# CloudEngineHub/FairyGen

Hardware: AMD Instinct MI355X
Metric: decoded frames/sec (sec/clip in config), Wan2.2-TI2V-5B 704x1280x121 @ 5 steps (higher is better)
Workload: dtype bf16

## Files before the change

fairygen_amd/csrc/capi.cpp:

```cpp
#include <stdarg.h>
#include <stdio.h>
#include "../../include/fairygen_hip.h"

static thread_local char g_err[512] = "";

void fg_set_error(const char* fmt, ...) {
    va_list ap;
    va_start(ap, fmt);
    vsnprintf(g_err, sizeof(g_err), fmt, ap);
    va_end(ap);
}

extern "C" int fg_version(void) { return 5; }
extern "C" const char* fg_last_error(void) { return g_err; }
```

fairygen_amd/csrc/dit_elementwise.hip:

```cpp
#include "common.h"

#ifndef FG_ROW_MIN_WAVES
#define FG_ROW_MIN_WAVES 4
#endif
#define FG_ROW_BOUNDS __launch_bounds__(256, FG_ROW_MIN_WAVES)

namespace {

constexpr int kMaxVec = 8;
constexpr int kRowsPerBlock = 4;

struct Row {
    float v[kMaxVec][8];
};

__device__ __forceinline__ void load_row(const bf16* p, int C, int lane, Row& r) {
    const int nvec = C >> 3;
#pragma unroll
    for (int i = 0; i < kMaxVec; ++i) {
        const int vi = lane + i * 64;
        if (vi < nvec) {
            bf16x8 t = *reinterpret_cast<const bf16x8*>(p + (int64_t)vi * 8);
#pragma unroll
            for (int j = 0; j < 8; ++j) r.v[i][j] = (float)t[j];
        } else {
#pragma unroll
            for (int j = 0; j < 8; ++j) r.v[i][j] = 0.f;
        }
    }
}

__device__ __forceinline__ bf16x8 ld8(const bf16* p) { return *reinterpret_cast<const bf16x8*>(p); }
__device__ __forceinline__ void st8(bf16* p, const float* f) {
    bf16x8 t;
#pragma unroll
    for (int j = 0; j < 8; ++j) t[j] = (bf16)f[j];
    *reinterpret_cast<bf16x8*>(p) = t;
}
// ... 238 lines not shown
                const int d0 = PLAIN ? ((vi * 8) & (head_dim - 1)) : ((vi * 8) % head_dim);
                if (F32TAB) {
                    f32x4 t0 = h0, t1 = h1;
                    if (!hoist) {
                        const f32x4* tp = reinterpret_cast<const f32x4*>(static_cast<const float*>(ctv) + (row * half + (d0 >> 1)) * 2);
                        t0 = tp[0];
                        t1 = tp[1];
                    }
                    const float cs[8] = {t0[0], t0[1], t0[2], t0[3], t1[0], t1[1], t1[2], t1[3]};
#pragma unroll
                    for (int j = 0; j < 4; ++j) {
                        const float a = o[2 * j], b = o[2 * j + 1], c = cs[2 * j], sn = cs[2 * j + 1];
                        o[2 * j] = rbf(__builtin_fmaf(a, c, -(b * sn)));
                        o[2 * j + 1] = rbf(__builtin_fmaf(a, sn, b * c));
                    }
                } else {
                    const double* cp = static_cast<const double*>(ctv) + row * half + (d0 >> 1);
                    const double* sp = static_cast<const double*>(stv) + row * half + (d0 >> 1);
#pragma unroll
                    for (int j = 0; j < 4; ++j) {
                        const double a = (double)o[2 * j], b = (double)o[2 * j + 1];
                        const double c = cp[j], sn = sp[j];
                        o[2 * j] = (float)(bf16)(a * c - b * sn);
                        o[2 * j + 1] = (float)(bf16)(a * sn + b * c);
                    }
                }
            }
            const int col = vi * 8, g = PLAIN ? 0 : col / group_cols;
            st8(out + g * out_group_stride + row * out_ld + (col - g * group_cols), o);
        }
    }
}

__global__ __launch_bounds__(256) void copy_groups_kernel(const bf16* __restrict__ src, int64_t sgs, int64_t sld,
                                                          bf16* __restrict__ dst, int64_t dgs, int64_t dld, int groups,
                                                          int64_t rows, int vec_per_row) {
    const int64_t total = (int64_t)groups * rows * vec_per_row;
    for (int64_t i = (int64_t)blockIdx.x * blockDim.x + threadIdx.x; i < total; i += (int64_t)gridDim.x * blockDim.x) {
        const int64_t rg = i / vec_per_row;
        const int v = (int)(i - rg * vec_per_row);
        const int64_t r = rg / groups;
        const int g = (int)(rg - r * groups);
        *reinterpret_cast<u32x4*>(dst + g * dgs + r * dld + v * 8) =
            *reinterpret_cast<const u32x4*>(src + g * sgs + r * sld + v * 8);
    }
}


template <int KIND>
__global__ __launch_bounds__(256) void act_kernel(const bf16* __restrict__ x, bf16* __restrict__ out, int64_t nvec) {
    for (int64_t i = (int64_t)blockIdx.x * blockDim.x + threadIdx.x; i < nvec; i += (int64_t)gridDim.x * blockDim.x) {
        const bf16x8 v = ld8(x + i * 8);
        float o[8];
#pragma unroll
        for (int j = 0; j < 8; ++j) o[j] = KIND == 0 ? silu_f((float)v[j]) : gelu_tanh_f((float)v[j]);
        st8(out + i * 8, o);
    }
}

__global__ __launch_bounds__(256) void cfg_euler_kernel(const bf16* __restrict__ lat, const bf16* __restrict__ posi,
                                                        const bf16* __restrict__ nega, bf16* __restrict__ out,
                                                        int64_t n, float cfg, float dsigma) {
    for (int64_t i = (int64_t)blockIdx.x * blockDim.x + threadIdx.x; i < n; i += (int64_t)gridDim.x * blockDim.x) {
        const float p = (float)posi[i];
        float pred = p;
        if (nega != nullptr) {
            const float ng = (float)nega[i];
            pred = rbf(ng + rbf(cfg * rbf(p - ng)));
        }
        out[i] = (bf16)((float)lat[i] + rbf(pred * dsigma));
    }
}

inline int check_rows(const char* fn, int64_t rows, int C, int64_t mod_rows, int64_t first_rows) {
    FG_CHECK_ARG(rows >= 0 && C > 0 && (C % 8) == 0 && C <= kMaxVec * 512, "%s: need C %% 8 == 0 and C <= %d (got rows=%lld C=%d)",
                 fn, kMaxVec * 512, (long long)rows, C);
    FG_CHECK_ARG(mod_rows == 1 || mod_rows == 2 || mod_rows == rows, "%s: mod_rows must be 1, 2 or rows (got %lld)", fn,
                 (long long)mod_rows);
    FG_CHECK_ARG(first_rows >= 0 && first_rows <= rows, "%s: first_rows out of range", fn);
    return FG_OK;
}

inline dim3 row_grid(int64_t rows) { return dim3((unsigned)((rows + kRowsPerBlock - 1) / kRowsPerBlock)); }

}

extern "C" {

int fg_ln_modulate_bf16(const void* x, const void* shift, const void* scale, void* out, int64_t rows, int C, float eps,
                        int64_t mod_rows, int64_t first_rows, int64_t mod_ld, fg_stream_t stream) {
    if (int e = check_rows("fg_ln_modulate_bf16", rows, C, mod_rows, first_rows)) return e;
    FG_CHECK_ARG(x && shift && scale && out, "fg_ln_modulate_bf16: null pointer");
    FG_CHECK_ARG(FG_ALIGNED16(x) && FG_ALIGNED16(shift) && FG_ALIGNED16(scale) && FG_ALIGNED16(out) && mod_ld % 8 == 0,
                 "fg_ln_modulate_bf16: pointers / mod_ld must be 16-byte aligned");
    if (rows == 0) return FG_OK;
    hipLaunchKernelGGL(ln_modulate_kernel, row_grid(rows), dim3(256), 0, (hipStream_t)stream, (const bf16*)x,
                       (const bf16*)shift, (const bf16*)scale, (bf16*)out, rows, C, eps, mod_rows, first_rows, mod_ld);
    return fg_launch_status("fg_ln_modulate_bf16");
}

int fg_ln_modulate_fp8_bf16(const void* x, const void* shift, const void* scale, void* out_fp8, float* out_scale, int64_t rows, int C,
                            float eps, int64_t mod_rows, int64_t first_rows, int64_t mod_ld, float fp8_max, fg_stream_t stream) {
    if (int e = check_rows("fg_ln_modulate_fp8_bf16", rows, C, mod_rows, first_rows)) return e;
    FG_CHECK_ARG(x && shift && scale && out_fp8 && out_scale, "fg_ln_modulate_fp8_bf16: null pointer");
    FG_CHECK_ARG(FG_ALIGNED16(x) && FG_ALIGNED16(shift) && FG_ALIGNED16(scale) && (((uintptr_t)out_fp8) & 7) == 0 && mod_ld % 8 == 0 &&
                     fp8_max > 0.f,
                 "fg_ln_modulate_fp8_bf16: pointers / mod_ld must be 16-byte aligned (out_fp8: 8), fp8_max positive");
    if (rows == 0) return FG_OK;
    hipLaunchKernelGGL(ln_modulate_fp8_kernel, row_grid(rows), dim3(256), 0, (hipStream_t)stream, (const bf16*)x, (const bf16*)shift,
                       (const bf16*)scale, (uint8_t*)out_fp8, out_scale, rows, C, eps, mod_rows, first_rows, mod_ld, fp8_max);
    return fg_launch_status("fg_ln_modulate_fp8_bf16");
}

int fg_ln_modulate_dual_bf16(const void* x, const void* shift, const void* scale, void* out, void* out_fp8, float* out_scale,
                             int64_t rows, int C, float eps, int64_t mod_rows, int64_t first_rows, int64_t mod_ld, float fp8_max,
                             fg_stream_t stream) {
    if (int e = check_rows("fg_ln_modulate_dual_bf16", rows, C, mod_rows, first_rows)) return e;
    FG_CHECK_ARG(x && shift && scale && out && out_fp8 && out_scale, "fg_ln_modulate_dual_bf16: null pointer");
    FG_CHECK_ARG(FG_ALIGNED16(x) && FG_ALIGNED16(shift) && FG_ALIGNED16(scale) && FG_ALIGNED16(out) && (((uintptr_t)out_fp8) & 7) == 0 &&
                     mod_ld % 8 == 0 && fp8_max > 0.f,
                 "fg_ln_modulate_dual_bf16: pointers / mod_ld must be 16-byte aligned (out_fp8: 8), fp8_max positive");
    if (rows == 0) return FG_OK;
    hipLaunchKernelGGL(ln_dual_kernel<0>, row_grid(rows), dim3(256), 0, (hipStream_t)stream, (const bf16*)x, (const bf16*)shift,
                       (const bf16*)scale, (bf16*)out, (uint8_t*)out_fp8, out_scale, rows, C, eps, mod_rows, first_rows, mod_ld, fp8_max);
    return fg_launch_status("fg_ln_modulate_dual_bf16");
}

int fg_ln_affine_dual_bf16(const void* x, const void* w, const void* b, void* out, void* out_fp8, float* out_scale, int64_t rows, int C,
// ... 9 lines not shown
    return fg_launch_status("fg_ln_affine_dual_bf16");
}

int fg_residual_ln_fp8_bf16(const void* x, const void* y, const void* gate, void* x_out, const void* p0, const void* p1,
                            void* norm_fp8, float* norm_scale, int mode, int64_t rows, int C, float eps, int64_t mod_rows,
                            int64_t first_rows, int64_t mod_ld, float fp8_max, fg_stream_t stream) {
    FG_CHECK_ARG(mode == 0 || mode == 1, "fg_residual_ln_fp8_bf16: mode must be 0 (modulate) or 1 (affine)");
    const bool need_mod = gate != nullptr || mode == 0;
    if (int e = check_rows("fg_residual_ln_fp8_bf16", rows, C, need_mod ? mod_rows : 1, need_mod ? first_rows : 0)) return e;
    FG_CHECK_ARG(x && y && x_out && p0 && p1 && norm_fp8 && norm_scale, "fg_residual_ln_fp8_bf16: null pointer");
    FG_CHECK_ARG(FG_ALIGNED16(x) && FG_ALIGNED16(y) && FG_ALIGNED16(gate) && FG_ALIGNED16(x_out) && FG_ALIGNED16(p0) &&
                     FG_ALIGNED16(p1) && (((uintptr_t)norm_fp8) & 7) == 0 && mod_ld % 8 == 0 && fp8_max > 0.f,
                 "fg_residual_ln_fp8_bf16: pointers / mod_ld must be 16-byte aligned (norm_fp8: 8), fp8_max positive");
    if (rows == 0) return FG_OK;
    if (!need_mod) { mod_rows = 1; first_rows = 0; }
    if (mode == 0)
        hipLaunchKernelGGL(residual_kernel<0>, row_grid(rows), dim3(256), 0, (hipStream_t)stream, (const bf16*)x,
                           (const bf16*)y, (const bf16*)gate, (bf16*)x_out, (const bf16*)p0, (const bf16*)p1,
                           (bf16*)nullptr, rows, C, eps, mod_rows, first_rows, mod_ld, (uint8_t*)norm_fp8, norm_scale, fp8_max);
    else
        hipLaunchKernelGGL(residual_kernel<1>, row_grid(rows), dim3(256), 0, (hipStream_t)stream, (const bf16*)x,
                           (const bf16*)y, (const bf16*)gate, (bf16*)x_out, (const bf16*)p0, (const bf16*)p1,
                           (bf16*)nullptr, rows, C, eps, mod_rows, first_rows, mod_ld, (uint8_t*)norm_fp8, norm_scale, fp8_max);
    return fg_launch_status("fg_residual_ln_fp8_bf16");
}

int fg_ln_affine_bf16(const void* x, const void* w, const void* b, void* out, int64_t rows, int C, float eps,
                      fg_stream_t stream) {
    if (int e = check_rows("fg_ln_affine_bf16", rows, C, 1, 0)) return e;
    FG_CHECK_ARG(x && w && b && out, "fg_ln_affine_bf16: null pointer");
    FG_CHECK_ARG(FG_ALIGNED16(x) && FG_ALIGNED16(w) && FG_ALIGNED16(b) && FG_ALIGNED16(out),
                 "fg_ln_affine_bf16: pointers must be 16-byte aligned");
    if (rows == 0) return FG_OK;
    hipLaunchKernelGGL(ln_affine_kernel, row_grid(rows), dim3(256), 0, (hipStream_t)stream, (const bf16*)x, (const bf16*)w,
                       (const bf16*)b, (bf16*)out, rows, C, eps);
    return fg_launch_status("fg_ln_affine_bf16");
}

int fg_gate_residual_bf16(const void* x, const void* y, const void* gate, void* out, int64_t rows, int C, int64_t mod_rows,
                          int64_t first_rows, int64_t mod_ld, fg_stream_t stream) {
    if (int e = check_rows("fg_gate_residual_bf16", rows, C, gate ? mod_rows : 1, gate ? first_rows : 0)) return e;
    FG_CHECK_ARG(x && y && out, "fg_gate_residual_bf16: null pointer");
    FG_CHECK_ARG(FG_ALIGNED16(x) && FG_ALIGNED16(y) && FG_ALIGNED16(gate) && FG_ALIGNED16(out) && mod_ld % 8 == 0,
                 "fg_gate_residual_bf16: pointers / mod_ld must be 16-byte aligned");
    if (rows == 0) return FG_OK;
    hipLaunchKernelGGL(residual_kernel<-1>, row_grid(rows), dim3(256), 0, (hipStream_t)stream, (const bf16*)x,
                       (const bf16*)y, (const bf16*)gate, (bf16*)out, (const bf16*)nullptr, (const bf16*)nullptr,
                       (bf16*)nullptr, rows, C, 0.f, gate ? mod_rows : 1, gate ? first_rows : 0, mod_ld);
    return fg_launch_status("fg_gate_residual_bf16");
}

int fg_residual_ln_bf16(const void* x, const void* y, const void* gate, void* x_out, const void* p0, const void* p1,
                        void* norm_out, int mode, int64_t rows, int C, float eps, int64_t mod_rows, int64_t first_rows,
                        int64_t mod_ld, fg_stream_t stream) {
    FG_CHECK_ARG(mode == 0 || mode == 1, "fg_residual_ln_bf16: mode must be 0 (modulate) or 1 (affine)");
    const bool need_mod = gate != nullptr || mode == 0;
    if (int e = check_rows("fg_residual_ln_bf16", rows, C, need_mod ? mod_rows : 1, need_mod ? first_rows : 0)) return e;
    FG_CHECK_ARG(x && y && x_out && p0 && p1 && norm_out, "fg_residual_ln_bf16: null pointer");
    FG_CHECK_ARG(FG_ALIGNED16(x) && FG_ALIGNED16(y) && FG_ALIGNED16(gate) && FG_ALIGNED16(x_out) && FG_ALIGNED16(p0) &&
                     FG_ALIGNED16(p1) && FG_ALIGNED16(norm_out) && mod_ld % 8 == 0,
                 "fg_residual_ln_bf16: pointers / mod_ld must be 16-byte aligned");
    if (rows == 0) return FG_OK;
    if (!need_mod) { mod_rows = 1; first_rows = 0; }
    if (mode == 0)
        hipLaunchKernelGGL(residual_kernel<0>, row_grid(rows), dim3(256), 0, (hipStream_t)stream, (const bf16*)x,
                           (const bf16*)y, (const bf16*)gate, (bf16*)x_out, (const bf16*)p0, (const bf16*)p1,
                           (bf16*)norm_out, rows, C, eps, mod_rows, first_rows, mod_ld);
    else
        hipLaunchKernelGGL(residual_kernel<1>, row_grid(rows), dim3(256), 0, (hipStream_t)stream, (const bf16*)x,
                           (const bf16*)y, (const bf16*)gate, (bf16*)x_out, (const bf16*)p0, (const bf16*)p1,
                           (bf16*)norm_out, rows, C, eps, mod_rows, first_rows, mod_ld);
    return fg_launch_status("fg_residual_ln_bf16");
}

int fg_rmsnorm_rope_bf16(const void* x, int64_t ldx, const void* weight, const void* cos_tab, const void* sin_tab,
                         int table_f32, void* out, int64_t rows, int C, int num_heads, float eps, fg_stream_t stream) {
    if (int e = check_rows("fg_rmsnorm_rope_bf16", rows, C, 1, 0)) return e;
    FG_CHECK_ARG(x && weight && out, "fg_rmsnorm_rope_bf16: null pointer");
    FG_CHECK_ARG(table_f32 ? (cos_tab != nullptr && sin_tab == nullptr) : ((cos_tab == nullptr) == (sin_tab == nullptr)),
                 "fg_rmsnorm_rope_bf16: fp64 mode takes both tables or neither, fp32 mode ONE interleaved table in cos_tab");
    FG_CHECK_ARG(num_heads > 0 && C % num_heads == 0 && (C / num_heads) % 8 == 0,
                 "fg_rmsnorm_rope_bf16: head_dim must be a multiple of 8");
    FG_CHECK_ARG(ldx >= C && ldx % 8 == 0 && FG_ALIGNED16(x) && FG_ALIGNED16(weight) && FG_ALIGNED16(out) &&
                     FG_ALIGNED16(cos_tab) && FG_ALIGNED16(sin_tab),
                 "fg_rmsnorm_rope_bf16: pointers / ldx must be 16-byte aligned");
    if (rows == 0) return FG_OK;
    const int hd = C / num_heads;
    const bool plain = (hd & (hd - 1)) == 0;
#define FG_ROPE_LAUNCH(TAB, PL)                                                                                                  \
    hipLaunchKernelGGL((rmsnorm_rope_kernel<TAB, PL>), row_grid(rows), dim3(256), 0, (hipStream_t)stream, (const bf16*)x, ldx,    \
                       (const bf16*)weight, cos_tab, sin_tab, (bf16*)out, rows, C, hd, eps, C, (int64_t)0, (int64_t)C)
    if (table_f32) { if (plain) FG_ROPE_LAUNCH(true, true); else FG_ROPE_LAUNCH(true, false); }
    else { if (plain) FG_ROPE_LAUNCH(false, true); else FG_ROPE_LAUNCH(false, false); }
#undef FG_ROPE_LAUNCH
    return fg_launch_status("fg_rmsnorm_rope_bf16");
}

int fg_rmsnorm_rope_grouped_bf16(const void* x, int64_t ldx, const void* weight, const void* cos_tab,
                                 const void* sin_tab, int table_f32, void* out, int64_t rows, int C, int num_heads, float eps,
                                 int group_cols, int64_t out_group_stride, int64_t out_ld, fg_stream_t stream) {
    if (int e = check_rows("fg_rmsnorm_rope_grouped_bf16", rows, C, 1, 0)) return e;
    FG_CHECK_ARG(x && weight && out, "fg_rmsnorm_rope_grouped_bf16: null pointer");
    FG_CHECK_ARG(table_f32 ? (cos_tab != nullptr && sin_tab == nullptr) : ((cos_tab == nullptr) == (sin_tab == nullptr)),
                 "fg_rmsnorm_rope_grouped_bf16: fp64 mode takes both tables or neither, fp32 mode ONE interleaved table in cos_tab");
    FG_CHECK_ARG(num_heads > 0 && C % num_heads == 0 && (C / num_heads) % 8 == 0,
                 "fg_rmsnorm_rope_grouped_bf16: head_dim must be a multiple of 8");
    FG_CHECK_ARG(group_cols > 0 && group_cols % 8 == 0 && C % group_cols == 0 && out_ld >= group_cols && out_ld % 8 == 0 &&
                     out_group_stride % 8 == 0 && out_group_stride >= 0,
                 "fg_rmsnorm_rope_grouped_bf16: group_cols must divide C; group_cols, out_ld, out_group_stride multiples of 8");
    FG_CHECK_ARG(ldx >= C && ldx % 8 == 0 && FG_ALIGNED16(x) && FG_ALIGNED16(weight) && FG_ALIGNED16(out) &&
                     FG_ALIGNED16(cos_tab) && FG_ALIGNED16(sin_tab),
                 "fg_rmsnorm_rope_grouped_bf16: pointers / ldx must be 16-byte aligned");
    if (rows == 0) return FG_OK;
    if (table_f32)
        hipLaunchKernelGGL((rmsnorm_rope_kernel<true, false>), row_grid(rows), dim3(256), 0, (hipStream_t)stream, (const bf16*)x, ldx,
                           (const bf16*)weight, cos_tab, sin_tab, (bf16*)out, rows, C, C / num_heads, eps, group_cols,
                           out_group_stride, out_ld);
    else
        hipLaunchKernelGGL((rmsnorm_rope_kernel<false, false>), row_grid(rows), dim3(256), 0, (hipStream_t)stream, (const bf16*)x, ldx,
                           (const bf16*)weight, cos_tab, sin_tab, (bf16*)out, rows, C, C / num_heads, eps, group_cols,
                           out_group_stride, out_ld);
    return fg_launch_status("fg_rmsnorm_rope_grouped_bf16");
}

int fg_copy_groups_bf16(const void* src, int64_t src_group_stride, int64_t src_ld, void* dst, int64_t dst_group_stride,
                        int64_t dst_ld, int groups, int64_t rows, int cols, fg_stream_t stream) {
    FG_CHECK_ARG(src && dst, "fg_copy_groups_bf16: null pointer");
    FG_CHECK_ARG(groups > 0 && rows >= 0 && cols > 0 && cols % 8 == 0, "fg_copy_groups_bf16: cols must be a positive multiple of 8");
// ... 37 lines not shown
```

fairygen_amd/hip.py:

```python
import ctypes
import os

import torch

_LIB_PATH = os.environ.get("FAIRYGEN_HIP_LIB") or os.path.join(os.path.dirname(os.path.abspath(__file__)), "libfairygen_hip.so")
_lib = None

ABI_VERSION = 5

_i64, _i32, _f32, _vp = ctypes.c_int64, ctypes.c_int, ctypes.c_float, ctypes.c_void_p

_SIGNATURES = {
    "fg_ln_modulate_bf16": [_vp, _vp, _vp, _vp, _i64, _i32, _f32, _i64, _i64, _i64, _vp],
    "fg_ln_affine_bf16": [_vp, _vp, _vp, _vp, _i64, _i32, _f32, _vp],
    "fg_ln_modulate_fp8_bf16": [_vp, _vp, _vp, _vp, _vp, _i64, _i32, _f32, _i64, _i64, _i64, _f32, _vp],
    "fg_residual_ln_fp8_bf16": [_vp, _vp, _vp, _vp, _vp, _vp, _vp, _vp, _i32, _i64, _i32, _f32, _i64, _i64, _i64, _f32, _vp],
    "fg_ln_modulate_dual_bf16": [_vp, _vp, _vp, _vp, _vp, _vp, _i64, _i32, _f32, _i64, _i64, _i64, _f32, _vp],
    "fg_ln_affine_dual_bf16": [_vp, _vp, _vp, _vp, _vp, _vp, _i64, _i32, _f32, _f32, _vp],
    "fg_gate_residual_bf16": [_vp, _vp, _vp, _vp, _i64, _i32, _i64, _i64, _i64, _vp],
    "fg_residual_ln_bf16": [_vp, _vp, _vp, _vp, _vp, _vp, _vp, _i32, _i64, _i32, _f32, _i64, _i64, _i64, _vp],
    "fg_rmsnorm_rope_bf16": [_vp, _i64, _vp, _vp, _vp, _i32, _vp, _i64, _i32, _i32, _f32, _vp],
    "fg_rmsnorm_rope_grouped_bf16": [_vp, _i64, _vp, _vp, _vp, _i32, _vp, _i64, _i32, _i32, _f32, _i32, _i64, _i64, _vp],
    "fg_copy_groups_bf16": [_vp, _i64, _i64, _vp, _i64, _i64, _i32, _i64, _i32, _vp],
    "fg_fp8_quant_rows_bf16": [_vp, _i64, _vp, _vp, _vp, _i64, _i32, _i32, _f32, _vp],
    "fg_act_bf16": [_vp, _vp, _i64, _i32, _vp],
    "fg_gemm_epilogue_bf16": [_vp, _i64, _vp, _vp, _vp, _i64, _i64, _i64, _i64, _i32, _vp, _i64, _i64, _i64, _vp, _vp],
    "fg_gemm_fp8_bf16": [_vp, _i64, _vp, _vp, _vp, _vp, _i64, _i64, _i64, _i64, _i32, _vp, _i64, _i64, _i64, _vp, _vp],
    "fg_lora_apply_bf16": [_vp, _i64, _vp, _vp, _vp, _i64, _i64, _i64, _i64, _i64, _i64, _i32, _vp, _i64, _i64, _i64, _vp],
    "fg_attn_fwd_bf16": [_vp, _i64, _vp, _i64, _vp, _i64, _vp, _i32, _i64, _i64, _i32, _i32, _f32, _vp, _i64, _vp],
    "fg_cfg_euler_bf16": [_vp, _vp, _vp, _vp, _i64, _f32, _f32, _vp],
    "fg_vae_rmsnorm_silu_bf16": [_vp, _vp, _vp, _i64, _i32, _i32, _vp],
    "fg_conv_pack_weight_bf16": [_vp, _vp, _i32, _i32, _i32, _i32, _i32, _vp],
    "fg_conv3d_cl_bf16": [_vp, _vp, _vp, _vp, _vp, _i32, _i32, _i32, _i32, _i32, _i32, _i32, _i32, _i32, _vp],
    "fg_dupup3d_add_bf16": [_vp, _vp, _vp, _i32, _i32, _i32, _i32, _i32, _i32, _i32, _i32, _vp],
    "fg_softmax_rows_f32_bf16": [_vp, _vp, _i64, _i64, _f32, _vp],
    "fg_vae_latent_to_cl_bf16": [_vp, _vp, _vp, _vp, _i32, _i32, _i32, _i32, _vp],
    "fg_vae_unpatchify_bf16": [_vp, _vp, _i32, _i32, _i32, _i32, _i32, _i32, _vp],
    "fg_vae_tile_accumulate_bf16": [_vp, _vp, _vp, _i32, _i32, _i32, _i32, _i32, _i32, _i32, _i32, _i32, _i32, _i32, _vp],
    "fg_vae_tile_finalize_bf16": [_vp, _vp, _i32, _i32, _i32, _i32, _i32, _vp],
    "fg_vae_patchify_bf16": [_vp, _vp, _i32, _i32, _i32, _vp],
    "fg_avgdown3d_add_bf16": [_vp, _vp, _vp, _i32, _i32, _i32, _i32, _i32, _i32, _i32, _vp],
    "fg_vae_latent_from_cl_bf16": [_vp, _vp, _vp, _vp, _i32, _i32, _i32, _i32, _i32, _vp],
    "fg_video_to_uint8": [_vp, _vp, _i32, _i32, _i32, _vp],
    "fg_softmax_bias_bf16": [_vp, _vp, _vp, _vp, _i64, _i64, _vp],
    "fg_gated_gelu_bf16": [_vp, _vp, _vp, _i64, _vp],
}
EXPORTED_SYMBOLS = sorted(list(_SIGNATURES) + ["fg_version", "fg_last_error", "fg_conv_packed_bytes", "fg_attn_workspace_bytes", "fg_attn_split_choice",
                                                   "fg_conv_tile_choice", "fg_gemm_workspace_bytes", "fg_gemm_debug_grid"])


class HipLibraryError(RuntimeError):
    pass


# ... 210 lines not shown
    x2 = x.reshape(-1, c) if x.is_contiguous() else x
    if x2.dim() != 2:
        x2 = x2.squeeze(0)
    if x2.dim() != 2:
        raise HipLibraryError("rmsnorm_rope: strided input must be 2-D (rows, C) or (1, rows, C)")
    rows, ld = x2.shape[0], x2.stride(0)
    if grouped is None:
        out = torch.empty(x.shape, dtype=x.dtype, device=x.device) if out is None else out
    f32tab = 0
    if cos is not None and sin is None:
        f32tab = 1
        _dev(cos, "rope table", torch.float32)
        if cos.shape != (rows, c // num_heads // 2, 2) or not cos.is_contiguous():
            raise HipLibraryError(f"rmsnorm_rope: the fp32 rope table must be ({rows}, {c // num_heads // 2}, 2) contiguous")
    elif cos is not None:
        _dev(cos, "cos", torch.float64), _dev(sin, "sin", torch.float64)
        if cos.shape != (rows, c // num_heads // 2) or not cos.is_contiguous() or not sin.is_contiguous():
            raise HipLibraryError(f"rmsnorm_rope: rope tables must be ({rows}, {c // num_heads // 2}) contiguous")
    if grouped is not None:
        dst, group_cols, group_stride, out_ld = grouped
        _dev(dst, "grouped dst")
        groups = c // group_cols
        if dst.dim() != 1 or dst.stride(0) != 1 or \
                (groups - 1) * group_stride + max(rows - 1, 0) * out_ld + group_cols > dst.numel():
            raise HipLibraryError("rmsnorm_rope: grouped destination too small for the requested layout")
        _call("fg_rmsnorm_rope_grouped_bf16", _ptr(x2), ld, _ptr(weight), _ptr(cos), _ptr(sin), f32tab, _ptr(dst), rows, c,
              num_heads, eps, group_cols, group_stride, out_ld, _stream(x))
        return dst
    _call("fg_rmsnorm_rope_bf16", _ptr(x2), ld, _ptr(weight), _ptr(cos), _ptr(sin), f32tab, _ptr(out), rows, c, num_heads,
          eps, _stream(x))
    return out


def copy_groups(src, src_group_stride, src_ld, dst, dst_group_stride, dst_ld, groups, rows, cols):
    _dev(src, "src"), _dev(dst, "dst")
    for t, gs, ld, name in ((src, src_group_stride, src_ld, "src"), (dst, dst_group_stride, dst_ld, "dst")):
        if t.dim() != 1 or t.stride(0) != 1 or (groups - 1) * gs + max(rows - 1, 0) * ld + cols > t.numel():
            raise HipLibraryError(f"copy_groups: {name} view too small for the requested layout")
    _call("fg_copy_groups_bf16", _ptr(src), src_group_stride, src_ld, _ptr(dst), dst_group_stride, dst_ld, groups, rows,
          cols, _stream(src))
    return dst


_gemm_workspace = {}


def _gemm_ws(x, m, n, k_bytes, workspace):
    tiles = ((m + 255) // 256) * (n // 256)
    need = load().fg_gemm_workspace_bytes(m, n, k_bytes) if workspace and (k_bytes // 128 >= 96 or tiles <= 8 * 256) else 0
    if need <= 0:
        return None
    key = (x.device, torch.cuda.current_stream(x.device).cuda_stream)
    ws = _gemm_workspace.get(key)
    if ws is None or ws.numel() < need:
        ws = _gemm_workspace[key] = torch.empty(need, dtype=torch.uint8, device=x.device)
    return ws


def _gemm_out(name, x, m, n, out, residual):
    if out is None:
        if residual:
            raise HipLibraryError(f"{name}: residual=True needs the contiguous residual stream as `out`")
        return torch.empty(x.shape[:-1] + (n,), dtype=torch.bfloat16, device=x.device)
    _dev(out, "out")
    if not out.is_contiguous() or out.numel() != m * n:
        raise HipLibraryError(f"{name}: `out` must be a contiguous bf16 tensor of {m} x {n} elements")
# ... 299 lines not shown
```

fairygen_amd/wan_video_dit.py:

```python
import math

import os

import torch
import torch.nn as nn
import torch.nn.functional as F

from . import hip, tuning


def sinusoidal_embedding_1d(dim, position):
    sinusoid = torch.outer(position.to(torch.float64),
                           torch.pow(10000.0, -torch.arange(dim // 2, dtype=torch.float64).div(dim // 2)))
    return torch.cat([sinusoid.cos(), sinusoid.sin()], dim=1).to(position.dtype)


def precompute_freqs_cis(dim, end=1024, theta=10000.0):
    freqs = 1.0 / (theta ** (torch.arange(0, dim, 2, device="cpu")[: dim // 2].double() / dim))
    freqs = torch.outer(torch.arange(end, device="cpu"), freqs)
    return torch.polar(torch.ones_like(freqs), freqs)


def precompute_freqs_cis_3d(dim, end=1024, theta=10000.0):
    return (precompute_freqs_cis(dim - 2 * (dim // 3), end, theta),
# ... 297 lines not shown
        wmat = self.patch_embedding.weight.view(self.dim, -1)
        return F.linear(cols, wmat, self.patch_embedding.bias), (f, h, w)

    def unpatchify(self, x, grid_size):
        f, h, w = grid_size
        px, py, pz = self.patch_size
        b = x.shape[0]
        x = x.view(b, f, h, w, px, py, pz, self.out_dim).permute(0, 7, 1, 4, 2, 5, 3, 6)
        return x.reshape(b, self.out_dim, f * px, h * py, w * pz)

    def _self_attention_steps(self, i, blk, mod, x, h, cos, sin, shard, shard_total, own, lin, hip_hot=False):
        c, nh, eps = self.dim, self.num_heads, self.eps
        fp8 = self.fp8_dtype if lin is not None else None
        hot = bool(self.hot_loras)
        sharded = shard is not None and shard.active
        wqkv, bqkv, _, _ = blk.fused_weights()
        sa = blk.self_attn
        hot8 = hip_hot and fp8 is not None
        if hot8:
            h, h8 = h
            qkv = lin(h8, 0, bqkv)
        elif fp8 is not None:
            qkv = lin(h, 0, bqkv)
        elif GEMM_BACKEND == "all" and own_gemm_ok(h.shape[1], 3 * c, c):
            qkv = gemm_bias_own(h, wqkv, bqkv)
        else:
            qkv = gemm_bias(h, wqkv, bqkv)
        if hot:
            self._hot_apply(tuple(f"blocks.{i}.self_attn.{nm}" for nm in "qkv"), h, qkv, hip_hot and (not hot8 or fp8_own_ok(3 * c, c)))
        v = qkv[..., 2 * c:]
        rk, rq = ((cos, None), (sin, None)) if cos.dtype == torch.float32 else ((cos, sin), (cos, sin))
        scale = self.attn_scale()[0]
        if not sharded:
            k = hip.rmsnorm_rope(qkv[..., c:2 * c], sa.norm_k.weight, nh, eps, *rk)
            q = hip.rmsnorm_rope(qkv[..., :c], sa.norm_q.weight, nh, eps, *rq)
            a = sa.attn(q, k, v) if scale is None else sa.attn(q, k, v, scale=scale)
        elif shard.attn_mode == "ulysses":
            n_loc, p_, size = x.shape[1], shard.world_size, shard.chunk(shard_total)
            g = c // nh * shard.heads_local(nh)
            send = shard.ulysses_send_buffer(shard_total, c, qkv, n_loc)
            flat, layout = send.view(-1), (g, size * 3 * g, 3 * g)
            hip.rmsnorm_rope(qkv[..., :c], sa.norm_q.weight, nh, eps, *rq, grouped=(flat, *layout))
            hip.rmsnorm_rope(qkv[..., c:2 * c], sa.norm_k.weight, nh, eps, *rk, grouped=(flat[g:], *layout))
            hip.copy_groups(qkv.view(-1)[2 * c:], g, 3 * c, flat[2 * g:], size * 3 * g, 3 * g, p_, n_loc, g)
            pending = shard.ulysses_exchange_async(send, shard_total)
            yield i
            qg, kg, vg = pending.wait()
            o_full = shard.ulysses_out_buffer(shard_total, g, qkv)
            hip.attention(qg, kg, vg, shard.heads_local(nh), out=o_full[:shard_total].unsqueeze(0), scale=scale)
            pending = shard.ulysses_out_async(o_full, shard_total, n_loc)
            yield i
            a = torch.empty((1, n_loc, c), dtype=qkv.dtype, device=qkv.device)
            hip.copy_groups(pending.wait_blocks().view(-1), size * g, g, a.view(-1), g, c, p_, n_loc, g)
        else:
            k = hip.rmsnorm_rope(qkv[..., c:2 * c], sa.norm_k.weight, nh, eps, *rk)
            pending = shard.all_gather_kv_async(k, v, shard_total)
            q = hip.rmsnorm_rope(qkv[..., :c], sa.norm_q.weight, nh, eps, *rq)
            yield i
            k, v = pending.wait()
            a = sa.attn(q, k, v) if scale is None else sa.attn(q, k, v, scale=scale)
        if hot8:
            x = self._fp8_hot_residual(f"blocks.{i}.self_attn.o", a, blk.fp8_weights(fp8)[1], sa.o.bias, x, mod, 2)
            return x, hip.ln_affine_dual(x, blk.norm3.weight, blk.norm3.bias, eps)
        pk = self._hot_pack((f"blocks.{i}.self_attn.o",)) if hip_hot else None
        if own and own_gemm_ok(a.shape[1], c, c) and pk is not False:
            x = gemm_residual(x, a, sa.o.weight, sa.o.bias, mod, 2)
            if pk:
                hip.lora_apply(a, pk[0], pk[1], x, mode="gate", mod=mod, gate_idx=2)
# ... 178 lines not shown
```

include/fairygen_hip.h:

```cpp
#ifndef FAIRYGEN_HIP_H
#define FAIRYGEN_HIP_H

#include <stdint.h>

#ifdef __cplusplus
extern "C" {
#endif

#define FG_OK        0
#define FG_EINVAL   (-1)
#define FG_ELAUNCH  (-2)

typedef void* fg_stream_t;

int         fg_version(void);
const char* fg_last_error(void);


int fg_ln_modulate_bf16(const void* x, const void* shift, const void* scale, void* out,
                        int64_t rows, int C, float eps,
                        int64_t mod_rows, int64_t first_rows, int64_t mod_ld, fg_stream_t stream);

int fg_ln_affine_bf16(const void* x, const void* w, const void* b, void* out,
                      int64_t rows, int C, float eps, fg_stream_t stream);
// ... 8 lines not shown
                        int64_t mod_rows, int64_t first_rows, int64_t mod_ld, fg_stream_t stream);

int fg_ln_modulate_fp8_bf16(const void* x, const void* shift, const void* scale, void* out_fp8, float* out_scale,
                            int64_t rows, int C, float eps, int64_t mod_rows, int64_t first_rows, int64_t mod_ld,
                            float fp8_max, fg_stream_t stream);
int fg_residual_ln_fp8_bf16(const void* x, const void* y, const void* gate, void* x_out, const void* p0, const void* p1,
                            void* norm_fp8, float* norm_scale, int mode, int64_t rows, int C, float eps,
                            int64_t mod_rows, int64_t first_rows, int64_t mod_ld, float fp8_max, fg_stream_t stream);

int fg_ln_modulate_dual_bf16(const void* x, const void* shift, const void* scale, void* out, void* out_fp8, float* out_scale,
                             int64_t rows, int C, float eps, int64_t mod_rows, int64_t first_rows, int64_t mod_ld,
                             float fp8_max, fg_stream_t stream);
int fg_ln_affine_dual_bf16(const void* x, const void* w, const void* b, void* out, void* out_fp8, float* out_scale,
                           int64_t rows, int C, float eps, float fp8_max, fg_stream_t stream);

int64_t fg_gemm_workspace_bytes(int64_t M, int64_t N, int64_t K);
int fg_gemm_epilogue_bf16(const void* a, int64_t lda, const void* w, const void* bias, void* c, int64_t ldc,
                          int64_t M, int64_t N, int64_t K, int mode, const void* gate, int64_t gate_rows, int64_t gate_ld,
                          int64_t first_rows, void* workspace, fg_stream_t stream);

int fg_lora_apply_bf16(const void* x, int64_t ldx, const void* a, const void* b, void* out, int64_t ldc, int64_t M, int64_t K,
                       int64_t Ng, int64_t R, int64_t G, int mode, const void* gate, int64_t gate_rows, int64_t gate_ld,
                       int64_t first_rows, fg_stream_t stream);

int fg_gemm_debug_grid(int workgroups);

int fg_gemm_fp8_bf16(const void* a_fp8, int64_t lda, const float* scale_a, const void* w_fp8, const void* bias, void* c, int64_t ldc,
                     int64_t M, int64_t N, int64_t K, int mode, const void* gate, int64_t gate_rows, int64_t gate_ld,
                     int64_t first_rows, void* workspace, fg_stream_t stream);

int fg_rmsnorm_rope_bf16(const void* x, int64_t ldx, const void* weight,
                         const void* cos_tab, const void* sin_tab, int table_f32, void* out,
                         int64_t rows, int C, int num_heads, float eps, fg_stream_t stream);

int fg_rmsnorm_rope_grouped_bf16(const void* x, int64_t ldx, const void* weight,
                                 const void* cos_tab, const void* sin_tab, int table_f32, void* out,
                                 int64_t rows, int C, int num_heads, float eps,
                                 int group_cols, int64_t out_group_stride, int64_t out_ld, fg_stream_t stream);

int fg_copy_groups_bf16(const void* src, int64_t src_group_stride, int64_t src_ld,
                        void* dst, int64_t dst_group_stride, int64_t dst_ld,
                        int groups, int64_t rows, int cols, fg_stream_t stream);

int fg_fp8_quant_rows_bf16(const void* x, int64_t ldx, void* out_fp8, float* scale, void* act_out,
                           int64_t rows, int C, int act, float fp8_max, fg_stream_t stream);

int fg_act_bf16(const void* x, void* out, int64_t n, int kind, fg_stream_t stream);

int64_t fg_attn_workspace_bytes(int B, int64_t Nq, int64_t Nkv, int H);
int fg_attn_split_choice(int B, int64_t Nq, int64_t Nkv, int H, int64_t workspace_bytes, int* R, int* S);
int fg_attn_fwd_bf16(const void* q, int64_t ldq, const void* k, int64_t ldk, const void* v, int64_t ldv,
                     void* out, int B, int64_t Nq, int64_t Nkv, int H, int D, float scale,
                     void* workspace, int64_t workspace_bytes, fg_stream_t stream);

int fg_cfg_euler_bf16(const void* latents, const void* posi, const void* nega, void* out,
                      int64_t n, float cfg_scale, float dsigma, fg_stream_t stream);


int fg_vae_rmsnorm_silu_bf16(const void* x, const void* gamma, void* out,
                             int64_t pixels, int C, int apply_silu, fg_stream_t stream);

int64_t fg_conv_packed_bytes(int Cout, int Cin, int kt, int kh, int kw);
int fg_conv_pack_weight_bf16(const void* w, void* packed, int Cout, int Cin, int kt, int kh, int kw,
                             fg_stream_t stream);

int fg_conv3d_cl_bf16(const void* x, const void* w_packed, const void* bias,
// ... 46 lines not shown
```

Baseline: 15.52.

## Add persistent streaming row kernels for LayerNorm and fused Q/K RMSNorm-RoPE

Adds persistent grid-stride kernels for LN-modulate, LN-affine and RMSNorm+RoPE at widths 1536/3072. Each block stages the modulation or weight vectors in shared memory once and prefetches the next row while reducing the current one. A new paired entry point normalises K and Q in a single launch, and the DiT self-attention path uses it when fp32 rope tables are present. This targets launch overhead, redundant parameter loads and memory latency, at the cost of more specialised code paths and a grid capped at a fixed number of blocks per CU.

```diff
diff --git a/fairygen_amd/csrc/capi.cpp b/fairygen_amd/csrc/capi.cpp
--- a/fairygen_amd/csrc/capi.cpp
+++ b/fairygen_amd/csrc/capi.cpp
@@ -11,5 +11,5 @@
     va_end(ap);
 }
 
-extern "C" int fg_version(void) { return 5; }
+extern "C" int fg_version(void) { return 6; }
 extern "C" const char* fg_last_error(void) { return g_err; }
diff --git a/fairygen_amd/csrc/dit_elementwise.hip b/fairygen_amd/csrc/dit_elementwise.hip
--- a/fairygen_amd/csrc/dit_elementwise.hip
+++ b/fairygen_amd/csrc/dit_elementwise.hip
@@ -4,6 +4,10 @@
 #define FG_ROW_MIN_WAVES 4
 #endif
 #define FG_ROW_BOUNDS __launch_bounds__(256, FG_ROW_MIN_WAVES)
+#ifndef FG_STREAM_MIN_WAVES
+#define FG_STREAM_MIN_WAVES 4
+#endif
+#define FG_STREAM_BOUNDS __launch_bounds__(256, FG_STREAM_MIN_WAVES)
 
 namespace {
 
@@ -308,6 +312,187 @@
     }
 }
 
+template <int NV>
+struct RawRow {
+    bf16x8 v[NV];
+};
+
+template <int NV>
+__device__ __forceinline__ void load_raw(const bf16* p, int lane, RawRow<NV>& r) {
+#pragma unroll
+    for (int i = 0; i < NV; ++i) r.v[i] = ld8(p + (lane + i * 64) * 8);
+}
+
+template <int NV>
+__device__ __forceinline__ void fill_params(bf16x8* dst, const bf16* src, bool one_plus) {
+    constexpr int K = (NV * 64 + 255) / 256;
+    constexpr int N = NV * 64, kWrap = N >= 256 ? 256 : 64;
+    static_assert((N >= 256 && N <= 512) || N == 192, "fill_params: 192 vectors, or 256 .. 512");
+    bf16x8 a[K];
+    int t[K];
+#pragma unroll
+    for (int k = 0; k < K; ++k) {
+        t[k] = threadIdx.x + k * 256;
+        if (t[k] >= N) t[k] -= kWrap;
+        a[k] = ld8(src + t[k] * 8);
+    }
+#pragma unroll
+    for (int k = 0; k < K; ++k) {
+        if (one_plus) {
+#pragma unroll
+            for (int j = 0; j < 8; ++j) a[k][j] = (bf16)(1.0f + (float)a[k][j]);
+        }
+        dst[t[k]] = a[k];
+    }
+}
+
+template <int MODE, int NV>
+__global__ FG_STREAM_BOUNDS void ln_stream_kernel(const bf16* __restrict__ x, const bf16* __restrict__ p0, const bf16* __restrict__ p1,
+                                               bf16* __restrict__ out, int64_t rows, float eps, int mod_rows, int64_t first_rows,
+                                               int64_t mod_ld) {
+    constexpr int C = NV * 512;
+    __shared__ bf16x8 par[2][2][NV * 64];
+    fill_params<NV>(par[0][0], p0, false);
+    fill_params<NV>(par[0][1], p1, MODE == 0);
+    if (mod_rows == 2) {
+        fill_params<NV>(par[1][0], p0 + mod_ld, false);
+        fill_params<NV>(par[1][1], p1 + mod_ld, MODE == 0);
+    }
+    __syncthreads();
+    const int lane = threadIdx.x & 63;
+    const int64_t stride = (int64_t)gridDim.x * kRowsPerBlock;
+    int64_t row = (int64_t)blockIdx.x * kRowsPerBlock + (threadIdx.x >> 6);
+    if (row >= rows) return;
+    RawRow<NV> raw;
+    load_raw<NV>(x + row * C, lane, raw);
+    for (; row < rows; row += stride) {
+        float v[NV][8];
+#pragma unroll
+        for (int i = 0; i < NV; ++i)
+#pragma unroll
+            for (int j = 0; j < 8; ++j) v[i][j] = (float)raw.v[i][j];
+        if (row + stride < rows) load_raw<NV>(x + (row + stride) * C, lane, raw);
+        float s = 0.f;
+#pragma unroll
+        for (int i = 0; i < NV; ++i)
+#pragma unroll
+            for (int j = 0; j < 8; ++j) s += v[i][j];
+        const float mean = wave_sum(s) / (float)C;
+        float q = 0.f;
+#pragma unroll
+        for (int i = 0; i < NV; ++i)
+#pragma unroll
+            for (int j = 0; j < 8; ++j) {
+                const float d = v[i][j] - mean;
+                q += d * d;
+            }
+        const float var = wave_sum(q) / (float)C;
+        const float rstd = 1.0f / sqrtf(var + eps);
+        asm volatile("" ::: "memory");
+        const int m = mod_rows == 2 && row >= first_rows ? 1 : 0;
+#pragma unroll
+        for (int i = 0; i < NV; ++i) {
+            const int vi = lane + i * 64;
+            const bf16x8 a = par[m][0][vi];
+            const bf16x8 b = par[m][1][vi];
+            float o[8];
+#pragma unroll
+            for (int j = 0; j < 8; ++j) {
+                const float n = (v[i][j] - mean) * rstd;
+                if (MODE == 0) {
+                    const float y = rbf(n);
+                    const float s1 = (float)b[j];
+                    o[j] = rbf(y * s1) + (float)a[j];
+                } else {
+                    float t = n * (float)a[j] + (float)b[j];
+                    asm volatile("" : "+v"(t));
+                    o[j] = t;
+                }
+            }
+            st8(out + row * C + vi * 8, o);
+        }
+    }
+}
+
+struct RopeOperand {
+    const bf16* x;
+    int64_t ldx;
+    const bf16* w;
+    const float* tab;
+    bf16* out;
+};
+struct RopeOperands {
+    RopeOperand op[2];
+};
+
+template <int NOPS, int NV>
+__global__ FG_STREAM_BOUNDS void rmsnorm_rope_stream_kernel(RopeOperands ops, int64_t rows, int head_dim, float eps) {
+    constexpr int C = NV * 512;
+    __shared__ bf16x8 wts[NOPS][NV * 64];
+#pragma unroll
+    for (int k = 0; k < NOPS; ++k) fill_params<NV>(wts[k], ops.op[k].w, false);
+    __syncthreads();
+    const int lane = threadIdx.x & 63;
+    const int64_t items = rows * NOPS;
+    const int64_t stride = (int64_t)gridDim.x * kRowsPerBlock;
+    int64_t it = (int64_t)blockIdx.x * kRowsPerBlock + (threadIdx.x >> 6);
+    if (it >= items) return;
+    const int half = head_dim >> 1;
+    const int d_lane = (lane * 8) & (head_dim - 1);
+    RawRow<NV> raw;
+    {
+        const RopeOperand o = ops.op[NOPS == 1 ? 0 : (int)(it & 1)];
+        load_raw<NV>(o.x + (it / NOPS) * o.ldx, lane, raw);
+    }
+    for (; it < items; it += stride) {
+        const int k = NOPS == 1 ? 0 : (int)(it & 1);
+        const int64_t row = it / NOPS;
+        const RopeOperand o = ops.op[k];
+        f32x4 h0 = {0.f, 0.f, 0.f, 0.f}, h1 = {0.f, 0.f, 0.f, 0.f};
+        if (o.tab != nullptr) {
+            const f32x4* tp = reinterpret_cast<const f32x4*>(o.tab + (row * half + (d_lane >> 1)) * 2);
+            h0 = tp[0];
+            h1 = tp[1];
+        }
+        float v[NV][8];
+#pragma unroll
+        for (int i = 0; i < NV; ++i)
+#pragma unroll
+            for (int j = 0; j < 8; ++j) v[i][j] = (float)raw.v[i][j];
+        if (it + stride < items) {
+            const int64_t nt = it + stride;
+            const RopeOperand n = ops.op[NOPS == 1 ? 0 : (int)(nt & 1)];
+            load_raw<NV>(n.x + (nt / NOPS) * n.ldx, lane, raw);
+        }
+        float q = 0.f;
+#pragma unroll
+        for (int i = 0; i < NV; ++i)
+#pragma unroll
+            for (int j = 0; j < 8; ++j) q += v[i][j] * v[i][j];
+        const float ms = wave_sum(q) / (float)C;
+        const float rinv = 1.0f / sqrtf(ms + eps);
+        const float cs[8] = {h0[0], h0[1], h0[2], h0[3], h1[0], h1[1], h1[2], h1[3]};
+        asm volatile("" ::: "memory");
+#pragma unroll
+        for (int i = 0; i < NV; ++i) {
+            const int vi = lane + i * 64;
+            const bf16x8 wv = wts[k][vi];
+            float r[8];
+#pragma unroll
+            for (int j = 0; j < 8; ++j) r[j] = rbf(rbf(v[i][j] * rinv) * (float)wv[j]);
+            if (o.tab != nullptr) {
+#pragma unroll
+                for (int j = 0; j < 4; ++j) {
+                    const float a = r[2 * j], b = r[2 * j + 1], c = cs[2 * j], sn = cs[2 * j + 1];
+                    r[2 * j] = rbf(__builtin_fmaf(a, c, -(b * sn)));
+                    r[2 * j + 1] = rbf(__builtin_fmaf(a, sn, b * c));
+                }
+            }
+            st8(o.out + row * C + vi * 8, r);
+        }
+    }
+}
+
 __global__ __launch_bounds__(256) void copy_groups_kernel(const bf16* __restrict__ src, int64_t sgs, int64_t sld,
                                                           bf16* __restrict__ dst, int64_t dgs, int64_t dld, int groups,
                                                           int64_t rows, int vec_per_row) {
@@ -359,6 +544,22 @@
 
 inline dim3 row_grid(int64_t rows) { return dim3((unsigned)((rows + kRowsPerBlock - 1) / kRowsPerBlock)); }
 
+inline dim3 stream_grid(int64_t items) {
+    static int cached_dev = -1, cached_cus = 256;
+    int dev = 0;
+    if (hipGetDevice(&dev) == hipSuccess && dev != cached_dev) {
+        int n = 0;
+        cached_cus = hipDeviceGetAttribute(&n, hipDeviceAttributeMultiprocessorCount, dev) == hipSuccess && n > 0 ? n : 256;
+        cached_dev = dev;
+    }
+    const int64_t need = (items + kRowsPerBlock - 1) / kRowsPerBlock, slots = (int64_t)cached_cus * FG_STREAM_MIN_WAVES;
+    return dim3((unsigned)(need < slots ? need : slots));
+}
+
+inline bool stream_width(int C) { return C == 1536 || C == 3072; }
+
+#define FG_STREAM_NV(C, LAUNCH) do { if ((C) == 1536) { LAUNCH(3); } else { LAUNCH(6); } } while (0)
+
 }
 
 extern "C" {
@@ -370,6 +571,14 @@
     FG_CHECK_ARG(FG_ALIGNED16(x) && FG_ALIGNED16(shift) && FG_ALIGNED16(scale) && FG_ALIGNED16(out) && mod_ld % 8 == 0,
                  "fg_ln_modulate_bf16: pointers / mod_ld must be 16-byte aligned");
     if (rows == 0) return FG_OK;
+    if (stream_width(C) && mod_rows <= 2) {
+#define FG_LAUNCH(NV)                                                                                                            \
+    hipLaunchKernelGGL((ln_stream_kernel<0, NV>), stream_grid(rows), dim3(256), 0, (hipStream_t)stream, (const bf16*)x,          \
+                       (const bf16*)shift, (const bf16*)scale, (bf16*)out, rows, eps, (int)mod_rows, first_rows, mod_ld)
+        FG_STREAM_NV(C, FG_LAUNCH);
+#undef FG_LAUNCH
+        return fg_launch_status("fg_ln_modulate_bf16");
+    }
     hipLaunchKernelGGL(ln_modulate_kernel, row_grid(rows), dim3(256), 0, (hipStream_t)stream, (const bf16*)x,
                        (const bf16*)shift, (const bf16*)scale, (bf16*)out, rows, C, eps, mod_rows, first_rows, mod_ld);
     return fg_launch_status("fg_ln_modulate_bf16");
@@ -445,6 +654,14 @@
     FG_CHECK_ARG(FG_ALIGNED16(x) && FG_ALIGNED16(w) && FG_ALIGNED16(b) && FG_ALIGNED16(out),
                  "fg_ln_affine_bf16: pointers must be 16-byte aligned");
     if (rows == 0) return FG_OK;
+    if (stream_width(C)) {
+#define FG_LAUNCH(NV)                                                                                                            \
+    hipLaunchKernelGGL((ln_stream_kernel<1, NV>), stream_grid(rows), dim3(256), 0, (hipStream_t)stream, (const bf16*)x,          \
+                       (const bf16*)w, (const bf16*)b, (bf16*)out, rows, eps, 1, (int64_t)0, (int64_t)0)
+        FG_STREAM_NV(C, FG_LAUNCH);
+#undef FG_LAUNCH
+        return fg_launch_status("fg_ln_affine_bf16");
+    }
     hipLaunchKernelGGL(ln_affine_kernel, row_grid(rows), dim3(256), 0, (hipStream_t)stream, (const bf16*)x, (const bf16*)w,
                        (const bf16*)b, (bf16*)out, rows, C, eps);
     return fg_launch_status("fg_ln_affine_bf16");
@@ -500,6 +717,14 @@
     if (rows == 0) return FG_OK;
     const int hd = C / num_heads;
     const bool plain = (hd & (hd - 1)) == 0;
+    if (stream_width(C) && plain && hd <= 512 && (table_f32 || cos_tab == nullptr)) {
+        const RopeOperands ops = {{{(const bf16*)x, ldx, (const bf16*)weight, (const float*)cos_tab, (bf16*)out}, {}}};
+#define FG_LAUNCH(NV)                                                                                                            \
+    hipLaunchKernelGGL((rmsnorm_rope_stream_kernel<1, NV>), stream_grid(rows), dim3(256), 0, (hipStream_t)stream, ops, rows, hd, eps)
+        FG_STREAM_NV(C, FG_LAUNCH);
+#undef FG_LAUNCH
+        return fg_launch_status("fg_rmsnorm_rope_bf16");
+    }
 #define FG_ROPE_LAUNCH(TAB, PL)                                                                                                  \
     hipLaunchKernelGGL((rmsnorm_rope_kernel<TAB, PL>), row_grid(rows), dim3(256), 0, (hipStream_t)stream, (const bf16*)x, ldx,    \
                        (const bf16*)weight, cos_tab, sin_tab, (bf16*)out, rows, C, hd, eps, C, (int64_t)0, (int64_t)C)
@@ -507,6 +732,30 @@
     else { if (plain) FG_ROPE_LAUNCH(false, true); else FG_ROPE_LAUNCH(false, false); }
 #undef FG_ROPE_LAUNCH
     return fg_launch_status("fg_rmsnorm_rope_bf16");
+}
+
+int fg_rmsnorm_rope_pair_bf16(const void* x0, const void* x1, int64_t ldx, const void* weight0, const void* weight1, const void* tab0,
+                              const void* tab1, void* out0, void* out1, int64_t rows, int C, int num_heads, float eps,
+                              fg_stream_t stream) {
+    if (int e = check_rows("fg_rmsnorm_rope_pair_bf16", rows, C, 1, 0)) return e;
+    FG_CHECK_ARG(x0 && x1 && weight0 && weight1 && out0 && out1 && out0 != out1, "fg_rmsnorm_rope_pair_bf16: null pointer");
+    FG_CHECK_ARG((tab0 == nullptr) == (tab1 == nullptr), "fg_rmsnorm_rope_pair_bf16: both operands rotate (fp32 tables) or neither");
+    FG_CHECK_ARG(num_heads > 0 && C % num_heads == 0, "fg_rmsnorm_rope_pair_bf16: C must be a multiple of num_heads");
+    const int hd = C / num_heads;
+    FG_CHECK_ARG(stream_width(C) && hd >= 8 && hd <= 512 && (hd & (hd - 1)) == 0,
+                 "fg_rmsnorm_rope_pair_bf16: needs C = 1536 or 3072 and a power-of-two head_dim in [8, 512] (got C=%d, head_dim=%d); "
+                 "call fg_rmsnorm_rope_bf16 per operand otherwise", C, hd);
+    FG_CHECK_ARG(ldx >= C && ldx % 8 == 0 && FG_ALIGNED16(x0) && FG_ALIGNED16(x1) && FG_ALIGNED16(weight0) && FG_ALIGNED16(weight1) &&
+                     FG_ALIGNED16(out0) && FG_ALIGNED16(out1) && FG_ALIGNED16(tab0) && FG_ALIGNED16(tab1),
+                 "fg_rmsnorm_rope_pair_bf16: pointers / ldx must be 16-byte aligned");
+    if (rows == 0) return FG_OK;
+    const RopeOperands ops = {{{(const bf16*)x0, ldx, (const bf16*)weight0, (const float*)tab0, (bf16*)out0},
+                               {(const bf16*)x1, ldx, (const bf16*)weight1, (const float*)tab1, (bf16*)out1}}};
+#define FG_LAUNCH(NV)                                                                                                            \
+    hipLaunchKernelGGL((rmsnorm_rope_stream_kernel<2, NV>), stream_grid(2 * rows), dim3(256), 0, (hipStream_t)stream, ops, rows, hd, eps)
+    FG_STREAM_NV(C, FG_LAUNCH);
+#undef FG_LAUNCH
+    return fg_launch_status("fg_rmsnorm_rope_pair_bf16");
 }
 
 int fg_rmsnorm_rope_grouped_bf16(const void* x, int64_t ldx, const void* weight, const void* cos_tab,
diff --git a/fairygen_amd/hip.py b/fairygen_amd/hip.py
--- a/fairygen_amd/hip.py
+++ b/fairygen_amd/hip.py
@@ -6,7 +6,7 @@
 _LIB_PATH = os.environ.get("FAIRYGEN_HIP_LIB") or os.path.join(os.path.dirname(os.path.abspath(__file__)), "libfairygen_hip.so")
 _lib = None
 
-ABI_VERSION = 5
+ABI_VERSION = 6
 
 _i64, _i32, _f32, _vp = ctypes.c_int64, ctypes.c_int, ctypes.c_float, ctypes.c_void_p
 
@@ -20,6 +20,7 @@
     "fg_gate_residual_bf16": [_vp, _vp, _vp, _vp, _i64, _i32, _i64, _i64, _i64, _vp],
     "fg_residual_ln_bf16": [_vp, _vp, _vp, _vp, _vp, _vp, _vp, _i32, _i64, _i32, _f32, _i64, _i64, _i64, _vp],
     "fg_rmsnorm_rope_bf16": [_vp, _i64, _vp, _vp, _vp, _i32, _vp, _i64, _i32, _i32, _f32, _vp],
+    "fg_rmsnorm_rope_pair_bf16": [_vp, _vp, _i64, _vp, _vp, _vp, _vp, _vp, _vp, _i64, _i32, _i32, _f32, _vp],
     "fg_rmsnorm_rope_grouped_bf16": [_vp, _i64, _vp, _vp, _vp, _i32, _vp, _i64, _i32, _i32, _f32, _i32, _i64, _i64, _vp],
     "fg_copy_groups_bf16": [_vp, _i64, _i64, _vp, _i64, _i64, _i32, _i64, _i32, _vp],
     "fg_fp8_quant_rows_bf16": [_vp, _i64, _vp, _vp, _vp, _i64, _i32, _i32, _f32, _vp],
@@ -296,6 +297,40 @@
     return out
 
 
+def rmsnorm_rope_pair_ok(c, num_heads):
+    hd = c // num_heads
+    return c in (1536, 3072) and c % num_heads == 0 and 8 <= hd <= 512 and hd & (hd - 1) == 0
+
+
+def rmsnorm_rope_pair(x0, x1, weight0, weight1, num_heads, eps, tab0=None, tab1=None):
+    _dev(x0, "x0"), _dev(x1, "x1"), _dev(weight0, "weight0"), _dev(weight1, "weight1")
+    c = x0.shape[-1]
+    xs = []
+    for x in (x0, x1):
+        if x.shape != x0.shape or x.stride(-1) != 1:
+            raise HipLibraryError("rmsnorm_rope_pair: operands must have one shape and a dense last dim")
+        x2 = x.reshape(-1, c) if x.is_contiguous() else x
+        x2 = x2.squeeze(0) if x2.dim() != 2 else x2
+        if x2.dim() != 2:
+            raise HipLibraryError("rmsnorm_rope_pair: strided input must be 2-D (rows, C) or (1, rows, C)")
+        xs.append(x2)
+    rows, ld = xs[0].shape[0], xs[0].stride(0)
+    if xs[1].stride(0) != ld and rows > 1:
+        raise HipLibraryError("rmsnorm_rope_pair: operands must share the leading dimension")
+    if (tab0 is None) != (tab1 is None):
+        raise HipLibraryError("rmsnorm_rope_pair: both operands take a rope table or neither")
+    for tab in (tab0, tab1):
+        if tab is not None:
+            _dev(tab, "rope table", torch.float32)
+            if tab.shape != (rows, c // num_heads // 2, 2) or not tab.is_contiguous():
+                raise HipLibraryError(f"rmsnorm_rope_pair: the fp32 rope table must be ({rows}, {c // num_heads // 2}, 2) contiguous")
+    out0 = torch.empty(x0.shape, dtype=x0.dtype, device=x0.device)
+    out1 = torch.empty(x0.shape, dtype=x0.dtype, device=x0.device)
+    _call("fg_rmsnorm_rope_pair_bf16", _ptr(xs[0]), _ptr(xs[1]), ld, _ptr(weight0), _ptr(weight1), _ptr(tab0), _ptr(tab1), _ptr(out0),
+          _ptr(out1), rows, c, num_heads, eps, _stream(x0))
+    return out0, out1
+
+
 def copy_groups(src, src_group_stride, src_ld, dst, dst_group_stride, dst_ld, groups, rows, cols):
     _dev(src, "src"), _dev(dst, "dst")
     for t, gs, ld, name in ((src, src_group_stride, src_ld, "src"), (dst, dst_group_stride, dst_ld, "dst")):
diff --git a/fairygen_amd/wan_video_dit.py b/fairygen_amd/wan_video_dit.py
--- a/fairygen_amd/wan_video_dit.py
+++ b/fairygen_amd/wan_video_dit.py
@@ -353,8 +353,11 @@
         rk, rq = ((cos, None), (sin, None)) if cos.dtype == torch.float32 else ((cos, sin), (cos, sin))
         scale = self.attn_scale()[0]
         if not sharded:
-            k = hip.rmsnorm_rope(qkv[..., c:2 * c], sa.norm_k.weight, nh, eps, *rk)
-            q = hip.rmsnorm_rope(qkv[..., :c], sa.norm_q.weight, nh, eps, *rq)
+            if cos.dtype == torch.float32 and hip.rmsnorm_rope_pair_ok(c, nh):
+                k, q = hip.rmsnorm_rope_pair(qkv[..., c:2 * c], qkv[..., :c], sa.norm_k.weight, sa.norm_q.weight, nh, eps, cos, sin)
+            else:
+                k = hip.rmsnorm_rope(qkv[..., c:2 * c], sa.norm_k.weight, nh, eps, *rk)
+                q = hip.rmsnorm_rope(qkv[..., :c], sa.norm_q.weight, nh, eps, *rq)
             a = sa.attn(q, k, v) if scale is None else sa.attn(q, k, v, scale=scale)
         elif shard.attn_mode == "ulysses":
             n_loc, p_, size = x.shape[1], shard.world_size, shard.chunk(shard_total)
diff --git a/include/fairygen_hip.h b/include/fairygen_hip.h
--- a/include/fairygen_hip.h
+++ b/include/fairygen_hip.h
@@ -64,6 +64,10 @@
 int fg_rmsnorm_rope_bf16(const void* x, int64_t ldx, const void* weight,
                          const void* cos_tab, const void* sin_tab, int table_f32, void* out,
                          int64_t rows, int C, int num_heads, float eps, fg_stream_t stream);
+
+int fg_rmsnorm_rope_pair_bf16(const void* x0, const void* x1, int64_t ldx, const void* weight0, const void* weight1,
+                              const void* tab0, const void* tab1, void* out0, void* out1,
+                              int64_t rows, int C, int num_heads, float eps, fg_stream_t stream);
 
 int fg_rmsnorm_rope_grouped_bf16(const void* x, int64_t ldx, const void* weight,
                                  const void* cos_tab, const void* sin_tab, int table_f32, void* out,
```

New measurement: 15.60, median of 6. About the same (+0.5%).
